# zhenyuw16/Uni3DETR

Hardware: AMD Instinct MI355X
Metric: scenes/sec (fwd+bwd) SUN-RGB-D 20k pts, 300 queries (higher is better)
Workload: dtype bf16

## Files before the change

### include/u3d_hip.h

```cpp
#ifndef U3D_HIP_H_
#define U3D_HIP_H_

#include <stddef.h>
#include <stdint.h>

#ifdef __cplusplus
extern "C" {
#endif

typedef struct ihipStream_t* u3d_stream;

enum {
  U3D_OK = 0,
  U3D_ERR_ARG = -1,
  U3D_ERR_UNSUPPORTED = -2,
  U3D_ERR_LAUNCH = -3,
  U3D_ERR_WORKSPACE = -4
};

enum { U3D_F32 = 0, U3D_BF16 = 1 };

int32_t u3d_version(void);
const char* u3d_strerror(int32_t code);

// ... 59 lines not shown
                             const float voxel_size[3], const float pc_range[6], int32_t* coors, u3d_stream s);
int32_t u3d_scatter_mean(const float* points, const int32_t* rank, int32_t n_total, int32_t nfeat, float* sums,
                         int32_t* counts, int32_t n_voxels, u3d_stream s);

int32_t u3d_spconv_fwd(const void* in, const void* w, const int32_t* nbr, int32_t ld, void* out,
                       const int32_t* n_out_dev, int32_t n_out_cap, int32_t cin, int32_t cout, int32_t kvol,
                       int32_t transpose_w, int32_t dtype, u3d_stream s);

enum { U3D_FWD_EPI_PLAIN, U3D_FWD_EPI_ADD, U3D_FWD_EPI_STATS, U3D_FWD_EPI_AFFINE, U3D_FWD_EPI_COUNT };
enum { U3D_FWD_FAM_NONE, U3D_FWD_FAM_CONV_IN, U3D_FWD_FAM_DIRECT, U3D_FWD_FAM_GLDS, U3D_FWD_FAM_REG, U3D_FWD_FAM_COUNT };
typedef struct u3d_fwd_plan_info {
  int32_t family, kernel, rows, cols, partials, rows_per_partial, takes_addend;
} u3d_fwd_plan_info;
int32_t u3d_igemm_fwd_plan(int32_t n_out_cap, int32_t cin, int32_t cout, int32_t kvol, int32_t has_nbr, int32_t nmajor, int32_t epi,
                           u3d_fwd_plan_info* info);
int32_t u3d_igemm_fwd_bf16(const void* in, const void* w, const int32_t* nbr, int32_t ld, void* out,
                           const int32_t* n_out_dev, int32_t n_out_cap, int32_t cin, int32_t cout, int32_t kvol,
                           int32_t transpose_w, const void* addend, double* stats, u3d_stream s);
int32_t u3d_linear_bf16(const void* x, const void* w, const float* bias, int32_t relu, void* out, const int32_t* m_dev,
                        int32_t m_cap, int32_t k, int32_t n, u3d_stream s);
typedef struct u3d_bn_fold_job {
  const float* w;
  const float* gamma;
  const float* beta;
  const float* mean;
  const float* var;
  uint16_t* w_folded;
  float* shift;
  int64_t sk, sa, sb;
  float eps;
// ... 128 lines not shown
                     const int32_t* n_dev, int32_t n_cap, int32_t c, int32_t dtype, const int32_t* row_map, const void* post_add,
                     u3d_stream s);
int32_t u3d_bn_bwd_stats(const void* dy, const void* y, const void* x, const float* mean, const float* invstd,
                         const float* gamma, const float* beta, int32_t relu, const int32_t* n_dev, int32_t n_cap,
                         int32_t c, int32_t dtype, double* sums, void* workspace, int64_t workspace_bytes,
                         const int32_t* row_map, float* sums_f32, u3d_stream s);
int32_t u3d_bn_bwd_apply(const void* dy, const void* y, const void* x, const float* mean, const float* invstd,
                         const float* gamma, const float* beta, const double* sums, int32_t relu, void* dx, void* dres,
                         const int32_t* n_dev, int32_t n_cap, int32_t c, int32_t dtype, const int32_t* row_map, u3d_stream s);
int32_t u3d_bn_apply_planes(const float* x, const float* mean, const float* invstd, const float* gamma, const float* beta,
                            const float* residual, int32_t relu, float* y, void* planes, const int32_t* n_dev, int32_t n_cap,
                            int32_t c, const int32_t* row_map, const float* post_add, u3d_stream s);
int32_t u3d_bn_bwd_apply_planes(const float* dy, const float* y, const float* x, const float* mean, const float* invstd,
                                const float* gamma, const float* beta, const double* sums, int32_t relu, float* dx, float* dres,
                                void* planes, const int32_t* n_dev, int32_t n_cap, int32_t c, const int32_t* row_map, u3d_stream s);

int32_t u3d_to_dense(const void* feat, const int32_t* coors, const int32_t* n_dev, int32_t n_cap, int32_t c,
                     void* dense, int32_t dz, int32_t dy, int32_t dx, int32_t dtype, u3d_stream s);
int32_t u3d_from_dense(const void* dense, const int32_t* coors, const int32_t* n_dev, int32_t n_cap, int32_t c,
                       void* feat, int32_t dz, int32_t dy, int32_t dx, int32_t dtype, u3d_stream s);

int32_t u3d_gather_rows(const void* in, const int32_t* idx, int32_t n, int32_t row_bytes, void* out, u3d_stream s);
int32_t u3d_scatter_rows(const void* in, const int32_t* idx, int32_t n, int32_t row_bytes, void* out, u3d_stream s);

int32_t u3d_fps(const float* base, const int64_t* set_off, const int32_t* set_n, int32_t nsets, int32_t max_n,
                int32_t m, int32_t* out_idx, float* temp, int64_t temp_stride, int32_t* err, int64_t poll_ticks, int32_t max_wg,
                u3d_stream s);
int32_t u3d_fps2(const float* base, const float* base2, int32_t split, const int64_t* set_off, const int32_t* set_n,
                 int32_t nsets, int32_t max_n, int32_t m, int32_t* out_idx, float* temp, int64_t temp_stride, int32_t* err,
                 int64_t poll_ticks, int32_t max_wg, u3d_stream s);
// ... 337 lines not shown
```

### uni3detr_amd/csrc/igemm_bf16.hip

```cpp
#include "igemm_common.h"
#include "conv_in.h"
#include "igemm_direct.h"

#ifndef IGEMM_SMALL_WM
#define IGEMM_SMALL_WM 4
#endif
#ifndef GLDS256_CFG
#define GLDS256_CFG 2, 4, 8, 4
#endif
#ifndef GLDS_DMA_SPREAD
#define GLDS_DMA_SPREAD 2
#endif
#ifndef GLDS_FRAG_B128
#define GLDS_FRAG_B128 1
#endif
#ifndef IGEMM_STORE_KS
#define IGEMM_STORE_KS 0
#endif

__device__ __forceinline__ bf16x8 direct_frag(const u16* tile, int stride, int r0, int k0, int lane) {
  const int g = lane >> 4, i = lane & 15;
  const u16* p = tile + (r0 + i) * stride + k0 + 4 * g;
  typedef const volatile s16x4 __attribute__((address_space(3))) * lds_vptr;
  s16x4 a = *(lds_vptr)(p);
// ... 835 lines not shown

struct FwdPlan {
  int family = U3D_FWD_FAM_NONE;
  int kernel = 0;
  DirectPlan direct;
  glds_kernel_t fn = nullptr;
  int rows = 0, cols = 0;
  dim3 grid;
  int threads = 0;
  size_t lds = 0;
  int partials = 0, part_rows = 0;
  bool addend = false;
  bool served() const { return family != U3D_FWD_FAM_NONE; }
};

constexpr int GLDS8N_MIN_KTILES = 48;
constexpr int GLDS8N_MIN_WGS = 160;

static FwdPlan fwd_plan(int n_out_cap, int cin, int cout, int kvol, bool has_nbr, bool nmajor, FwdEpi epi) {
  FwdPlan p;
  const bool plain = epi == EPI_PLAIN || epi == EPI_ADD;
  auto tiled = [&](int family, int kernel, int rows, int cols, int threads, size_t lds) {
    p.family = family, p.kernel = kernel, p.rows = rows, p.cols = cols, p.threads = threads, p.lds = lds;
    p.grid = dim3(u3d_cdiv(n_out_cap, rows), u3d_cdiv(cout, cols));
  };
  if (plain && !nmajor && convin_shape(cin, cout, kvol)) {
    tiled(U3D_FWD_FAM_CONV_IN, 0, 256, CONVIN_COUT, 256, 0);
    return p;
  }
  if (plain || epi == EPI_STATS) {
// ... 7 lines not shown
  }
  if (n_out_cap <= 0 || cin <= 0 || cout <= 0) return p;
  const long long tiles256 = u3d_cdiv(n_out_cap, 256);
  if (nmajor && cin % 64 == 0 && cout % 64 == 0) {
    const bool r192 = has_nbr && kvol > 1;
    int g;
    if (epi == EPI_BIAS_RELU)
      g = (cout % 256 == 0 && tiles256 * (cout / 256) >= 128) ? G_256x256
          : (cout % 128 == 0 && tiles256 * (cout / 128) >= 128) ? G_256x128 : G_128x64;
    else if (cout % 256 == 0 && tiles256 * (cout / 256) >= 128)
      g = !has_nbr ? G_256x256 : (r192 && igemm_rows192(n_out_cap, cout / 256)) ? G8_192x256 : G8_256x256;
    else if (has_nbr && cout % 128 == 0 && kvol * (cin / 64) >= GLDS8N_MIN_KTILES && tiles256 * (cout / 128) >= GLDS8N_MIN_WGS)
      g = (r192 && igemm_rows192(n_out_cap, cout / 128)) ? G8_192x128 : G8_256x128;
    else
      g = cout % 128 == 0 ? G_128x128 : G_128x64;
    const GldsKernel& k = GLDS_KERNELS[g];
    p.fn = (epi == EPI_F32 || epi == EPI_F32_ADD) ? k.f32 : k.bf16;
    if (!p.fn) return p;
    tiled(U3D_FWD_FAM_GLDS, g, k.rows, k.cols, k.threads, k.lds);
    p.partials = (int)p.grid.x;
    p.part_rows = k.rows;
    p.addend = k.addend;
    return p;
  }
  if (!plain) return p;
  int r = -1;
  if ((cin == 16 || cin == 32) && (cout == 16 || cout == 32 || cout == 64))
    r = (cout == 16 ? R_N16_K : cout == 32 ? R_N32_K : R_N64_K) + (nmajor ? 1 : 0);
  else if (!nmajor && cin % 64 == 0 && cout % 64 == 0)
    r = cout % 256 == 0 ? (tiles256 * (cout / 256) < 128 ? R_256x128 : R_256x256) : cout % 128 == 0 ? R_256x128 : R_128x64;
// ... 76 lines not shown
```

### uni3detr_amd/csrc/rowops.hip

```cpp
#include "common.h"
#include <type_traits>

typedef unsigned short u16;
__device__ __forceinline__ float ld_elem(const float* p, long long i) { return p[i]; }
__device__ __forceinline__ float ld_elem(const u16* p, long long i) { return __uint_as_float(((unsigned)p[i]) << 16); }
__device__ __forceinline__ void st_elem(float* p, long long i, float v) { p[i] = v; }
__device__ __forceinline__ void st_elem(u16* p, long long i, float v) {
  unsigned u = __float_as_uint(v);
  if ((u & 0x7fffffffu) > 0x7f800000u) { p[i] = (u16)((u >> 16) | 0x40u); return; }
  u += 0x7fffu + ((u >> 16) & 1u);
  p[i] = (u16)(u >> 16);
}

static inline int st_rows_per_block(int n_cap, int c) {
  if (n_cap >= 131072) return c >= 128 ? 256 : 512;
  return n_cap >= 32768 ? 128 : 16;
}

template <typename T> struct VecOf;
template <> struct VecOf<float> { static constexpr int N = 4; };
template <> struct VecOf<u16> { static constexpr int N = 8; };

template <typename T>
__device__ __forceinline__ void load_vec(const T* p, float* out);
// ... 14 lines not shown
template <int V>
__device__ __forceinline__ void load_cols(const float* __restrict__ p, int col0, float* out) {
#pragma unroll
  for (int i = 0; i < V; i += 4) {
    const float4 t = *(const float4*)(p + col0 + i);
    out[i] = t.x; out[i + 1] = t.y; out[i + 2] = t.z; out[i + 3] = t.w;
  }
}
template <int V>
__device__ __forceinline__ void load_cols_d(const double* __restrict__ p, int col0, float scale, float* out) {
#pragma unroll
  for (int i = 0; i < V; i += 2) {
    const double2 t = *(const double2*)(p + col0 + i);
    out[i] = (float)t.x * scale; out[i + 1] = (float)t.y * scale;
  }
}

template <typename T, int MODE>
__global__ __launch_bounds__(256) void k_col_stats_vec(const T* __restrict__ x, const T* __restrict__ dy, const T* __restrict__ y,
                                                       const float* __restrict__ mean, const float* __restrict__ invstd,
                                                       const float* __restrict__ gamma, const float* __restrict__ beta, int relu,
                                                       const int* __restrict__ n_dev, int n_cap, int c, double* __restrict__ partial,
                                                       const int* __restrict__ row_map, int rows_per_block) {
  constexpr int V = VecOf<T>::N;
  extern __shared__ __attribute__((aligned(16))) char smem_raw[];
  double* red = (double*)smem_raw;
  const int n = min(*n_dev, n_cap);
  const int cv = c / V;
  const int cw = cv < 256 ? cv : 256;
  const int rl = 256 / cw;
// ... 18 lines not shown
      for (int r = r0 + trow; r < r1; r += rl) {
        const long long o = (long long)r * c + (long long)vc * V;
        float xv[V];
        load_vec<T>(x + o, xv);
        if (MODE == 0) {
#pragma unroll
          for (int e = 0; e < V; ++e) { s0[e] += xv[e]; s1[e] += xv[e] * xv[e]; }
        } else {
          float gv[V], yv[V];
          const long long oy = row_map ? (long long)row_map[r] * c + (long long)vc * V : o;
          load_vec<T>(dy + oy, gv);
          if (relu && !remask) load_vec<T>(y + oy, yv);
#pragma unroll
          for (int e = 0; e < V; ++e) {
            float g = gv[e];
            if (remask) yv[e] = (xv[e] - mu[e]) * is[e] * ga[e] + be[e];
            if (relu && !(yv[e] > 0.f)) g = 0.f;
            s0[e] += g;
            s1[e] += g * ((xv[e] - mu[e]) * is[e]);
          }
        }
      }
    }
    const int ncol = cw * V;
    if (trow < rl) {
#pragma unroll
      for (int e = 0; e < V; ++e) {
        red[(0 * rl + trow) * ncol + tcol * V + e] = (double)s0[e];
        red[(1 * rl + trow) * ncol + tcol * V + e] = (double)s1[e];
      }
    }
// ... 479 lines not shown
                                                      const int* __restrict__ n_dev, int n_cap, int c, const int* __restrict__ row_map,
                                                      const T* __restrict__ post_add, u16* __restrict__ planes = nullptr) {
  constexpr int V = VecOf<T>::N;
  static_assert(!PLANES || V == 4, "planes are an f32 feature");
  const int n = min(*n_dev, n_cap), cv = c / V, rpb = 256 / cv;
  const int vc = threadIdx.x % cv, rl = threadIdx.x / cv;
  float mu[V], is[V], ga[V], be[V];
  load_cols<V>(mean, vc * V, mu); load_cols<V>(invstd, vc * V, is); load_cols<V>(gamma, vc * V, ga); load_cols<V>(beta, vc * V, be);
  for (int r = blockIdx.x * rpb + rl; r < n; r += gridDim.x * rpb) {
    const long long o = (long long)r * c + (long long)vc * V;
    float xv[V], rv[V], out[V];
    load_vec<T>(x + o, xv);
    if (res) load_vec<T>(res + o, rv);
#pragma unroll
    for (int e = 0; e < V; ++e) {
      float v = (xv[e] - mu[e]) * is[e] * ga[e] + be[e];
      if (res) v += rv[e];
      if (relu) v = v > 0.f ? v : 0.f;
      out[e] = v;
    }
    const long long oy = row_map ? (long long)row_map[r] * c + (long long)vc * V : o;
    if (post_add) {
      float pv[V];
      load_vec<T>(post_add + oy, pv);
#pragma unroll
      for (int e = 0; e < V; ++e) out[e] += pv[e];
    }
    store_vec<T>(y + oy, out);
    if constexpr (PLANES) store_planes4(planes + oy, (long long)n_cap * c, out);
  }
  if constexpr (PLANES) {
// ... 24 lines not shown
    for (int e = 0; e < V; ++e) be[e] = 0.f;
  }
  load_cols_d<V>(sums, vc * V, inv_n, mg);
  load_cols_d<V>(sums + c, vc * V, inv_n, mgx);
#pragma unroll 2
  for (int r = blockIdx.x * rpb + rl; r < n; r += gridDim.x * rpb) {
    const long long o = (long long)r * c + (long long)vc * V;
    float gv[V], xv[V], yv[V], dxv[V];
    const long long oy = row_map ? (long long)row_map[r] * c + (long long)vc * V : o;
    load_vec<T>(dy + oy, gv);
    load_vec<T>(x + o, xv);
    if (relu && !remask) load_vec<T>(y + oy, yv);
#pragma unroll
    for (int e = 0; e < V; ++e) {
      float g = gv[e];
      if (remask) yv[e] = (xv[e] - mu[e]) * is[e] * ga[e] + be[e];
      if (relu && !(yv[e] > 0.f)) g = 0.f;
      const float xh = (xv[e] - mu[e]) * is[e];
      dxv[e] = ga[e] * is[e] * (g - mg[e] - xh * mgx[e]);
      gv[e] = g;
    }
    store_vec<T>(dx + o, dxv);
    if constexpr (PLANES) store_planes4(planes + o, (long long)n_cap * c, dxv);
    if (dres) store_vec<T>(dres + o, gv);
  }
  if constexpr (PLANES) {
    const float z[4] = {0.f, 0.f, 0.f, 0.f};
    for (int r = n + blockIdx.x * rpb + rl; r < n_cap; r += gridDim.x * rpb)
      store_planes4(planes + (long long)r * c + (long long)vc * V, (long long)n_cap * c, z);
  }
}

static inline bool bn_vec_ok(int c, int v) { return c % v == 0 && (c / v) <= 256 && 256 % (c / v) == 0; }
static inline int bn_vec_grid(int n_cap, int c, int v) {
  int rpb = 256 / (c / v);
  long long b = ((long long)n_cap + rpb - 1) / rpb;
  return (int)(b < 1 ? 1 : (b > 2048 ? 2048 : b));
}

static inline int ew_grid(long long total) {
  long long b = (total + 255) / 256;
  return (int)(b < 1 ? 1 : (b > 8192 ? 8192 : b));
}

// ... 53 lines not shown
  U3D_CHECK_LAUNCH();
  return U3D_OK;
}
extern "C" int32_t u3d_bn_bwd_apply_planes(const float* dy, const float* y, const float* x, const float* mean, const float* invstd,
                                           const float* gamma, const float* beta, const double* sums, int32_t relu, float* dx, float* dres,
                                           void* planes, const int32_t* n_dev, int32_t n_cap, int32_t c, const int32_t* row_map, u3d_stream s) {
  U3D_REQUIRE(dy && x && mean && invstd && gamma && sums && dx && planes && n_dev && c > 0 && (!relu || y || beta), U3D_ERR_ARG);
  if (!bn_vec_ok(c, 4) || !(al16(mean) && al16(invstd) && al16(gamma) && al16(beta) && al16(sums)) || (row_map && dres)) return U3D_ERR_UNSUPPORTED;
  if (n_cap <= 0) return U3D_OK;
  hipLaunchKernelGGL((k_bn_bwd_apply_vec<float, true>), dim3(bn_vec_grid(n_cap, c, 4)), dim3(256), 0, s, dy, y, x, mean, invstd, gamma, beta, sums, relu,
                     dx, dres, n_dev, n_cap, c, row_map, (u16*)planes);
  U3D_CHECK_LAUNCH();
  return U3D_OK;
}

template <bool TO_DENSE>
__global__ void k_dense_rows(const uint32_t* __restrict__ src, const int4* __restrict__ coors, const int* __restrict__ n_dev,
                             int n_cap, int row_words, uint32_t* __restrict__ dst, int dz, int dy, int dx) {
  long long total = (long long)min(*n_dev, n_cap) * row_words;
  for (long long t = (long long)blockIdx.x * blockDim.x + threadIdx.x; t < total; t += (long long)gridDim.x * blockDim.x) {
    int r = (int)(t / row_words), w = (int)(t % row_words);
    int4 c = coors[r];
    long long cell = (((long long)c.x * dz + c.y) * dy + c.z) * dx + c.w;
    if (TO_DENSE) dst[cell * row_words + w] = src[t];
    else dst[t] = src[cell * row_words + w];
  }
}

static int run_dense(bool to_dense, const void* a, const int32_t* coors, const int32_t* n_dev, int n_cap, int c, void* b, int dz,
                     int dy, int dx, int dtype, hipStream_t s) {
// ... 320 lines not shown
```

### uni3detr_amd/native.py

```python
import collections
import ctypes as C
import os

import numpy as np
import torch

from . import abi

_HERE = os.path.dirname(os.path.abspath(__file__))
LIB_PATH = os.environ.get("U3D_LIB_PATH") or os.path.join(_HERE, "libu3d_hip.so")

_ABI = abi.load()
_K = _ABI.constants


def _struct(c_name, py_name):
    return abi.structure(_ABI.structs[c_name], py_name)


def _slot_names(prefix):
    names = sorted((v, n[len(prefix):]) for n, v in _K.items() if n.startswith(prefix))
    assert [v for v, _ in names] == list(range(len(names))) and names[-1][1] == "COUNT" and _K[prefix + "COUNT"] == len(names) - 1
    return [n for _, n in names[:-1]]


U3D_ERR_UNSUPPORTED = _K["U3D_ERR_UNSUPPORTED"]
F32, BF16 = _K["U3D_F32"], _K["U3D_BF16"]


class U3DError(RuntimeError):
    pass


BitGridStruct = _struct("u3d_bitgrid", "BitGridStruct")

for _n, _v in _K.items():
    if _n.startswith(("U3D_DL_", "U3D_DLN_")):
        globals()[_n[4:]] = _v
DS_NAMES = _slot_names("U3D_DS_")
DG_NAMES = _slot_names("U3D_DG_")
DecLayerParams = _struct("u3d_declayer_params", "DecLayerParams")
DecLayerDims = _struct("u3d_declayer_dims", "DecLayerDims")
# ... 283 lines not shown
                  "glds_128x64")
FWD_KERNELS = {"conv_in": ("conv_in",), "glds": AFFINE_KERNELS,
               "direct": tuple(f"{s}_{v}" for s in ("32x16", "32x32", "32x64", "64x16", "64x32") for v in ("k", "n", "ns", "nf")),
               "reg": ("n16_k", "n16_n", "n32_k", "n32_n", "n64_k", "n64_n", "256x256", "256x128", "128x64")}
FwdPlanInfo = _struct("u3d_fwd_plan_info", "FwdPlanInfo")
FwdPlan = collections.namedtuple("FwdPlan", "family kernel rows cols partials rows_per_partial takes_addend")


def fwd_plan(n_out, cin, cout, kvol, has_nbr, nmajor, epi="plain"):
    i = FwdPlanInfo()
    rc = lib().u3d_igemm_fwd_plan(n_out, cin, cout, kvol, bool(has_nbr), bool(nmajor), FWD_EPI[epi], C.byref(i))
    if rc:
        return None if rc == U3D_ERR_UNSUPPORTED else _check(rc, "igemm_fwd_plan")
    family = FWD_FAMILIES[i.family]
    return FwdPlan(family, FWD_KERNELS[family][i.kernel], i.rows, i.cols, i.partials, i.rows_per_partial, bool(i.takes_addend))


def fwd_stats_layout(n_out, cin, cout, kvol, has_nbr):
    p = fwd_plan(n_out, cin, cout, kvol, has_nbr, True, "stats")
    return p and (p.partials, p.rows_per_partial)


class SubmHalo:
    TILE = 128

    MAX_ROWS = 140 * 256 * 32

    def __init__(self, nbr_fwd, n_dev, n_cap):
        dev = nbr_fwd.device
        a, b, t = C.c_int64(0), C.c_int64(0), C.c_int32(0)
# ... 665 lines not shown
    if want_planes:
        if x.dtype == torch.float32 and x.is_cuda:
            planes = torch.empty((2 * n, c), dtype=torch.bfloat16, device=x.device)
            rc = lib().u3d_bn_bwd_apply_planes(_ptr(dy), _ptr(y), _ptr(x), _ptr(mean), _ptr(invstd), _ptr(gamma), _ptr(beta), _ptr(sums), int(relu),
                                               _ptr(dx), _ptr(dres), _ptr(planes), _ptr(n_dev), n, c, _ptr(row_map), _stream())
            if rc == 0:
                return dx, dres, planes
            if rc != U3D_ERR_UNSUPPORTED:
                _check(rc, "bn_bwd_apply_planes")
        _check(lib().u3d_bn_bwd_apply(_ptr(dy), _ptr(y), _ptr(x), _ptr(mean), _ptr(invstd), _ptr(gamma), _ptr(beta), _ptr(sums), int(relu),
                                      _ptr(dx), _ptr(dres), _ptr(n_dev), n, c, dtype_code(x), _ptr(row_map), _stream()), "bn_bwd_apply")
        return dx, dres, None
    _check(lib().u3d_bn_bwd_apply(_ptr(dy), _ptr(y), _ptr(x), _ptr(mean), _ptr(invstd), _ptr(gamma), _ptr(beta), _ptr(sums), int(relu),
                                  _ptr(dx), _ptr(dres), _ptr(n_dev), n, c, dtype_code(x), _ptr(row_map), _stream()), "bn_bwd_apply")
    return dx, dres


def to_dense(feat, coors, n_dev, batch, dims):
    n, c = feat.shape
    dz, dy, dx = dims
    vol = torch.zeros((batch, dz, dy, dx, c), dtype=feat.dtype, device=feat.device)
    _check(lib().u3d_to_dense(_ptr(feat), _ptr(coors), _ptr(n_dev), n, c, _ptr(vol), dz, dy, dx, dtype_code(feat), _stream()),
           "to_dense")
    return vol.permute(0, 4, 1, 2, 3)


def from_dense(vol_cl, coors, n_dev, n):
    b, dz, dy, dx, c = vol_cl.shape
    feat = torch.empty((n, c), dtype=vol_cl.dtype, device=vol_cl.device)
    _check(lib().u3d_from_dense(_ptr(vol_cl), _ptr(coors), _ptr(n_dev), n, c, _ptr(feat), dz, dy, dx, dtype_code(vol_cl),
# ... 1080 lines not shown
```

### uni3detr_amd/plugin/dense.py

```python

import numpy as np
import torch
from torch import nn

from .. import native as nv
from .. import sparse as sp
from ..registry import BACKBONES, NECKS


def _conv(cfg, cin, cout, kernel, stride=1, padding=0):
    cfg = dict(cfg)
    t = cfg.pop("type")
    if t != "Conv3d":
        raise NotImplementedError("the HIP dense path implements the Conv3d variant used by every shipped config")
    if cfg.get("bias", True):
        raise NotImplementedError("shipped configs build these convolutions with bias=False")
    return nn.Conv3d(cin, cout, kernel, stride=stride, padding=padding, **cfg)


def _norm(cfg, c):
    cfg = dict(cfg)
    t = cfg.pop("type")
    assert t == "BN3d", "shipped configs use BN3d"
    cfg.pop("requires_grad", None)
# ... 35 lines not shown
            z = torch.arange(D, device=device).view(1, -1, 1, 1)
            y = torch.arange(H * s, device=device).view(1, 1, -1, 1)
            x = torch.arange(W * s, device=device).view(1, 1, 1, -1)
            in_row = ((b * D + z) * H + y // s) * W + x // s
            tap = (y % s) * s + (x % s)
            idx = (in_row * (s * s) + tap).reshape(-1).int().contiguous()
            inv = torch.empty_like(idx)
            inv[idx.long()] = torch.arange(idx.numel(), device=device, dtype=torch.int32)
            v = (idx, inv, (D, H * s, W * s))
            cls._cache[key] = v
        return v


FUSED_LEVEL_SUM = True
FUSED_UPSAMPLE_ORDER = True


class _GatherBijection(torch.autograd.Function):
    @staticmethod
    def forward(ctx, rows, idx, inv):
        ctx.save_for_backward(inv)
        return nv.gather_rows(rows.contiguous(), idx)

    @staticmethod
    def backward(ctx, dout):
        (inv,) = ctx.saved_tensors
        return nv.gather_rows(dout.contiguous(), inv), None, None


def to_rows(x):
    B, C, D, H, W = x.shape
    return x.permute(0, 2, 3, 4, 1).reshape(-1, C), B, (D, H, W)


def to_volume(rows, B, dims):
    return rows.view(B, *dims, rows.shape[1]).permute(0, 4, 1, 2, 3)


def conv_bn_relu(rows, B, dims, conv, bn, post_add=None, fan_token=None):
    ks, st, pd = tuple(conv.kernel_size), tuple(conv.stride), tuple(conv.padding)
    geom, dims_out = Lattice.conv(rows.device, B, dims, ks, st, pd)
    return sp.conv_bn(rows, conv.weight, geom, bn, geom.n_out_dev, None, True, "oidhw", post_add, fan_token=fan_token), dims_out


def deconv_bn_relu(rows, B, dims, deconv, bn, post_add=None):
    s = deconv.stride[1]
    assert tuple(deconv.kernel_size) == (1, s, s) and tuple(deconv.stride) == (1, s, s), "non-overlapping (1,s,s) upsampling only"
    cin, cout = deconv.weight.shape[0], deconv.weight.shape[1]
    n_in = rows.shape[0]
    geom, _ = Lattice.conv(rows.device, B, dims, (1, 1, 1), (1, 1, 1), (0, 0, 0))
    w = deconv.weight.permute(0, 2, 3, 4, 1).reshape(1, 1, 1, cin, s * s * cout)
    y = sp.sparse_conv(rows, w, geom).view(n_in * s * s, cout)
    idx, inv, dims_out = Lattice.upsample_index(rows.device, B, dims, s)
    n_dev = Lattice.conv(rows.device, B, dims_out, (1, 1, 1), (1, 1, 1), (0, 0, 0))[0].n_out_dev
    if FUSED_UPSAMPLE_ORDER:
        return sp.bn_rows(y, bn, n_dev, None, True, row_map=inv, post_add=post_add), dims_out
    y = _GatherBijection.apply(y, idx, inv)
    return sp.bn_rows(y, bn, n_dev, None, True, post_add=post_add), dims_out


FANOUT_FUSION = True


@BACKBONES.register_module()
class SECOND3D(nn.Module):
    def __init__(self, in_channels=128, out_channels=[128, 128, 256], layer_nums=[3, 5, 5], layer_strides=[2, 2, 2],
                 is_cascade=True, norm_cfg=dict(type="BN3d", eps=1e-3, momentum=0.01), conv_cfg=dict(type="Conv3d", bias=False),
                 init_cfg=None, pretrained=None):
        super().__init__()
# ... 82 lines not shown
        self.deblocks = nn.ModuleList(deblocks)
        self.extra_conv = extra_conv
        if extra_conv is not None:
            extra = dict(extra_conv)
            self.layer_num = extra.pop("num_conv")
            kernel = tuple(extra.pop("kernel")) if "kernel" in extra else (3, 3, 3)
            if "sep_kernel" in extra:
                raise NotImplementedError("sep_kernel is not used by any shipped Uni3DETR config")
            padding = tuple((k - 1) // 2 for k in kernel)
            layers = []
            for _ in range(self.layer_num):
                layers += [_conv(extra, out_channels[-1], out_channels[-1], kernel, 1, padding), _norm(norm_cfg, out_channels[-1]),
                           nn.ReLU(inplace=True)]
            self.extra_blocks = nn.Sequential(*layers)

    def forward(self, x):
        assert len(x) == len(self.in_channels)
        out, odims, B = None, None, None
        for i, d in enumerate(self.deblocks):
            rows, B, dims = to_rows(x[i])
            fuse = FUSED_LEVEL_SUM and out is not None and rows.is_cuda and out.dtype == rows.dtype
            if isinstance(d[0], nn.ConvTranspose3d):
                r, dd = deconv_bn_relu(rows, B, dims, d[0], d[1], out if fuse else None)
            else:
                r, dd = conv_bn_relu(rows, B, dims, d[0], d[1], out if fuse else None)
            assert odims is None or odims == dd, "FPN levels must land on one lattice"
            out, odims = (r if (out is None or fuse) else out + r), dd
        if self.extra_conv is not None:
            mods = list(self.extra_blocks)
            for j in range(0, len(mods), 3):
                out, odims = conv_bn_relu(out, B, odims, mods[j], mods[j + 1])
        return to_volume(out, B, odims)
```

### uni3detr_amd/sparse.py

```python
import collections
import contextlib
import os

import torch

from . import native as nv
from .shadow import conv_weights, halo_packs

K3, S1, P1 = (3, 3, 3), (1, 1, 1), (1, 1, 1)


class Level:

    def __init__(self, grid, coords, n, n_dev):
        self.grid, self.coords, self.n, self.n_dev = grid, coords, n, n_dev
        self.dims, self.batch = grid.dims, grid.batch
        self._subm = None
        self._halo = None

    def halo(self):
        if self._halo is None:
            h = nv.SubmHalo(self.subm_tables()[0], self.n_dev, self.n) if self.n <= nv.SubmHalo.MAX_ROWS else None
            self._halo = h if (h is not None and h.ok) else False
        return self._halo or None
# ... 479 lines not shown
    kvol, cout, cin = ent.w_folded.shape
    halo = _halo_of(geom, kvol, cin, cout) if ent.route == "halo" else None
    if residual is not None and halo is None and ent.route != "direct":
        return None
    feats, add = feats.contiguous(), None if residual is None else residual.contiguous()
    nv.CALL_KIND = geom.kind
    if halo is not None:
        return nv.subm_halo_conv_affine(feats, ent.w_packed, halo, ent.shift, relu, add)
    if ent.route == "direct":
        return nv.igemm_direct_affine(feats, ent.w_folded, geom.nbr_fwd, ent.shift, relu, geom.n_out_dev, geom.n_out, add)
    if ent.route == "fp8":
        nv.absmax_rows(feats, geom.n_in_dev, ent.slot)
    return nv.igemm_fwd_affine(feats, ent.w_folded, geom.nbr_fwd if kvol > 1 else None, ent.shift, relu, geom.n_out_dev, geom.n_out)


def conv_bn(feats, weight, geom, bn, n_dev, residual=None, relu=True, layout="dhwio", post_add=None, res_take=None, res_give=None, fan_token=None):
    if _FOLD[0] is not None:
        ent = _FOLD[0].get(id(bn))
        if ent is not None:
            if bn.training or post_add is not None or (residual is not None and not ent.sparse_level):
                what = "an fp8 conv + BatchNorm pair" if ent.route == "fp8" else "a folded conv + BatchNorm pair"
                raise RuntimeError(f"{what} of a sparse level was called in training mode, or with a level sum" if ent.sparse_level else
                                   f"{what} was called in training mode, or with a residual / level sum")
            y = conv_folded(feats, ent, geom, residual, relu)
            if y is not None:
                return y
    if FUSED_CONV_STATS and bn.training and feats.is_cuda and (feats.dtype == torch.bfloat16 or _split_serves(feats, feats.shape[1], bn.num_features) == "wide"):
        y, stats = _SparseConv.apply(feats, weight, geom, layout, True, res_take, fan_token)
        if stats.numel():
            tr = getattr(stats, "_u3d_tile_rows", None)
            if tr is None:
                nb = stats.shape[0]
                tr = next((t for t in (128, 256, 192) if (y.shape[0] + t - 1) // t == nb), 0)
            return _BNRows.apply(y, bn.weight, bn.bias, residual, n_dev, bn, relu, True, stats, tr, None, post_add, res_give)
        return _BNRows.apply(y, bn.weight, bn.bias, residual, n_dev, bn, relu, bn.training, None, 0, None, post_add, res_give)
    return bn_rows(sparse_conv(feats, weight, geom, layout, fan_token), bn, n_dev, residual, relu, None, post_add)


class _BNRows(torch.autograd.Function):

    @staticmethod
    def forward(ctx, x, gamma, beta, residual, n_dev, bn, relu, training, stats=None, tile_rows=0, row_map=None, post_add=None, res_token=None):
        n = x.shape[0]
        if training and stats is not None:
            mean, invstd = nv.bn_finalize_partials(stats, tile_rows, n_dev, n, bn.eps, bn.momentum if bn.momentum is not None else 0.1,
                                                   bn.running_mean, bn.running_var, bn.num_batches_tracked)
        elif training:
            mean, invstd = nv.bn_forward_stats(x, n_dev, bn.eps, bn.momentum if bn.momentum is not None else 0.1,
                                               bn.running_mean, bn.running_var, bn.num_batches_tracked)
        else:
# ... 28 lines not shown
            dx, dres, dpl = nv.bn_bwd_apply(dy, y, x, mean, invstd, gamma, use, ctx.relu, ctx.n_dev, ctx.has_res, beta, ctx.row_map, want_planes=True)
            _give_bwd_planes(dx, dpl)
        else:
            dx, dres = nv.bn_bwd_apply(dy, y, x, mean, invstd, gamma, use, ctx.relu, ctx.n_dev, ctx.has_res, beta, ctx.row_map)
        if ctx.pdtype != torch.float32:
            s32 = s32.to(ctx.pdtype)
        if ctx.res_token is not None and dres is not None:
            ctx.res_token.dres, dres = dres, None
        return dx, s32[1], s32[0], dres, None, None, None, None, None, None, None, (dy if ctx.has_post else None), None


def bn_rows(x, bn, n_dev, residual=None, relu=True, row_map=None, post_add=None):
    return _BNRows.apply(x, bn.weight, bn.bias, residual, n_dev, bn, relu, bn.training, None, 0, row_map, post_add, None)


class _ToDense(torch.autograd.Function):
    @staticmethod
    def forward(ctx, feats, lvl):
        ctx.lvl = lvl
        vol = nv.to_dense(feats, lvl.coords, lvl.n_dev, lvl.batch, lvl.dims)
        ctx.active = _ACTIVE[0] = None
        if ACTIVE_FIRST_CONV and ctx.needs_input_grad[0] and feats.dtype == torch.bfloat16 and feats.is_cuda:
            ctx.set_materialize_grads(False)
            ctx.active = _ACTIVE[0] = ActiveInput(lvl, feats, vol)
        return vol

    @staticmethod
    def backward(ctx, dvol):
        lvl, act = ctx.lvl, ctx.active
        din = None
# ... 42 lines not shown
```

Before: 438.6.

## Fuse FPN level BN-apply, ReLU and sum into one multi-level kernel

Adds kernels that apply BatchNorm and ReLU to up to four FPN levels and sum them in a single pass, plus a matching backward kernel that writes every level's input gradient from one read of the upstream gradient. The neck forward now routes through this merged path in training, so it no longer runs a separate BN-apply and add per level. This cuts separate launches and intermediate activation round-trips through memory, at the cost of holding every level's input for backward. It also adds a short-K kernel override hook for 1x1 convs, which stays inactive unless it is selected.

```diff
diff --git a/include/u3d_hip.h b/include/u3d_hip.h
--- a/include/u3d_hip.h
+++ b/include/u3d_hip.h
@@ -97,6 +97,8 @@
 } u3d_fwd_plan_info;
 int32_t u3d_igemm_fwd_plan(int32_t n_out_cap, int32_t cin, int32_t cout, int32_t kvol, int32_t has_nbr, int32_t nmajor, int32_t epi,
                            u3d_fwd_plan_info* info);
+#define U3D_SHORT_K_PLAN -1
+int32_t u3d_igemm_short_k_select(int32_t kernel);
 int32_t u3d_igemm_fwd_bf16(const void* in, const void* w, const int32_t* nbr, int32_t ld, void* out,
                            const int32_t* n_out_dev, int32_t n_out_cap, int32_t cin, int32_t cout, int32_t kvol,
                            int32_t transpose_w, const void* addend, double* stats, u3d_stream s);
@@ -255,6 +257,14 @@
 int32_t u3d_bn_bwd_apply_planes(const float* dy, const float* y, const float* x, const float* mean, const float* invstd,
                                 const float* gamma, const float* beta, const double* sums, int32_t relu, float* dx, float* dres,
                                 void* planes, const int32_t* n_dev, int32_t n_cap, int32_t c, const int32_t* row_map, u3d_stream s);
+#define U3D_BN_LEVELS_MAX 4
+int32_t u3d_bn_apply_levels(const void* const* x, const float* const* mean, const float* const* invstd, const float* const* gamma,
+                            const float* const* beta, const int32_t* const* src_map, int32_t levels, void* y, const int32_t* n_dev,
+                            int32_t n_cap, int32_t c, int32_t dtype, u3d_stream s);
+int32_t u3d_bn_bwd_apply_levels(const void* dout, const void* const* x, const float* const* mean, const float* const* invstd,
+                                const float* const* gamma, const float* const* beta, const double* const* sums,
+                                const int32_t* const* src_map, void* const* dx, int32_t levels, const int32_t* n_dev, int32_t n_cap,
+                                int32_t c, int32_t dtype, u3d_stream s);
 
 int32_t u3d_to_dense(const void* feat, const int32_t* coors, const int32_t* n_dev, int32_t n_cap, int32_t c,
                      void* dense, int32_t dz, int32_t dy, int32_t dx, int32_t dtype, u3d_stream s);
diff --git a/uni3detr_amd/csrc/igemm_bf16.hip b/uni3detr_amd/csrc/igemm_bf16.hip
--- a/uni3detr_amd/csrc/igemm_bf16.hip
+++ b/uni3detr_amd/csrc/igemm_bf16.hip
@@ -873,6 +873,13 @@
   bool served() const { return family != U3D_FWD_FAM_NONE; }
 };
 
+static int g_short_k = U3D_SHORT_K_PLAN;
+extern "C" int32_t u3d_igemm_short_k_select(int32_t kernel) {
+  U3D_REQUIRE(kernel == U3D_SHORT_K_PLAN || kernel == G_256x256 || kernel == G_256x128 || kernel == G_128x128 || kernel == G_128x64, U3D_ERR_ARG);
+  g_short_k = kernel;
+  return U3D_OK;
+}
+
 constexpr int GLDS8N_MIN_KTILES = 48;
 constexpr int GLDS8N_MIN_WGS = 160;
 
@@ -910,6 +917,9 @@
       g = (r192 && igemm_rows192(n_out_cap, cout / 128)) ? G8_192x128 : G8_256x128;
     else
       g = cout % 128 == 0 ? G_128x128 : G_128x64;
+    if (g_short_k != U3D_SHORT_K_PLAN && !has_nbr && kvol == 1 && cin <= 512 && (plain || epi == EPI_STATS) &&
+        cout % GLDS_KERNELS[g_short_k].cols == 0)
+      g = g_short_k;
     const GldsKernel& k = GLDS_KERNELS[g];
     p.fn = (epi == EPI_F32 || epi == EPI_F32_ADD) ? k.f32 : k.bf16;
     if (!p.fn) return p;
diff --git a/uni3detr_amd/csrc/rowops.hip b/uni3detr_amd/csrc/rowops.hip
--- a/uni3detr_amd/csrc/rowops.hip
+++ b/uni3detr_amd/csrc/rowops.hip
@@ -52,6 +52,12 @@
     const double2 t = *(const double2*)(p + col0 + i);
     out[i] = (float)t.x * scale; out[i + 1] = (float)t.y * scale;
   }
+}
+
+__device__ __forceinline__ float bn_affine(float x, float mu, float is, float ga, float be) { return (x - mu) * is * ga + be; }
+__device__ __forceinline__ float bn_dx(float g, float x, float mu, float is, float ga, float mg, float mgx) {
+  const float xh = (x - mu) * is;
+  return ga * is * (g - mg - xh * mgx);
 }
 
 template <typename T, int MODE>
@@ -100,7 +106,7 @@
 #pragma unroll
           for (int e = 0; e < V; ++e) {
             float g = gv[e];
-            if (remask) yv[e] = (xv[e] - mu[e]) * is[e] * ga[e] + be[e];
+            if (remask) yv[e] = bn_affine(xv[e], mu[e], is[e], ga[e], be[e]);
             if (relu && !(yv[e] > 0.f)) g = 0.f;
             s0[e] += g;
             s1[e] += g * ((xv[e] - mu[e]) * is[e]);
@@ -610,7 +616,7 @@
     if (res) load_vec<T>(res + o, rv);
 #pragma unroll
     for (int e = 0; e < V; ++e) {
-      float v = (xv[e] - mu[e]) * is[e] * ga[e] + be[e];
+      float v = bn_affine(xv[e], mu[e], is[e], ga[e], be[e]);
       if (res) v += rv[e];
       if (relu) v = v > 0.f ? v : 0.f;
       out[e] = v;
@@ -665,10 +671,9 @@
 #pragma unroll
     for (int e = 0; e < V; ++e) {
       float g = gv[e];
-      if (remask) yv[e] = (xv[e] - mu[e]) * is[e] * ga[e] + be[e];
+      if (remask) yv[e] = bn_affine(xv[e], mu[e], is[e], ga[e], be[e]);
       if (relu && !(yv[e] > 0.f)) g = 0.f;
-      const float xh = (xv[e] - mu[e]) * is[e];
-      dxv[e] = ga[e] * is[e] * (g - mg[e] - xh * mgx[e]);
+      dxv[e] = bn_dx(g, xv[e], mu[e], is[e], ga[e], mg[e], mgx[e]);
       gv[e] = g;
     }
     store_vec<T>(dx + o, dxv);
@@ -679,6 +684,119 @@
     const float z[4] = {0.f, 0.f, 0.f, 0.f};
     for (int r = n + blockIdx.x * rpb + rl; r < n_cap; r += gridDim.x * rpb)
       store_planes4(planes + (long long)r * c + (long long)vc * V, (long long)n_cap * c, z);
+  }
+}
+
+template <typename T>
+__device__ __forceinline__ void round_vec(float* v);
+template <>
+__device__ __forceinline__ void round_vec<float>(float*) {}
+template <>
+__device__ __forceinline__ void round_vec<u16>(float* v) {
+  typedef float f32x8_t __attribute__((ext_vector_type(8)));
+  typedef __bf16 bf16x8_t __attribute__((ext_vector_type(8)));
+  const f32x8_t f = {v[0], v[1], v[2], v[3], v[4], v[5], v[6], v[7]};
+  const f32x8_t g = __builtin_convertvector(__builtin_convertvector(f, bf16x8_t), f32x8_t);
+#pragma unroll
+  for (int e = 0; e < 8; ++e) v[e] = g[e];
+}
+
+struct BnLevelsFwd {
+  const void* x[U3D_BN_LEVELS_MAX];
+  const float *mean[U3D_BN_LEVELS_MAX], *invstd[U3D_BN_LEVELS_MAX], *gamma[U3D_BN_LEVELS_MAX], *beta[U3D_BN_LEVELS_MAX];
+  const int* src_map[U3D_BN_LEVELS_MAX];
+};
+struct BnLevelsBwd {
+  const void* x[U3D_BN_LEVELS_MAX];
+  const float *mean[U3D_BN_LEVELS_MAX], *invstd[U3D_BN_LEVELS_MAX], *gamma[U3D_BN_LEVELS_MAX], *beta[U3D_BN_LEVELS_MAX];
+  const double* sums[U3D_BN_LEVELS_MAX];
+  const int* src_map[U3D_BN_LEVELS_MAX];
+  void* dx[U3D_BN_LEVELS_MAX];
+};
+
+template <typename T, int L>
+__global__ __launch_bounds__(256) void k_bn_apply_levels(BnLevelsFwd p, T* __restrict__ y, const int* __restrict__ n_dev, int n_cap, int c) {
+  constexpr int V = VecOf<T>::N;
+  const int n = min(*n_dev, n_cap), cv = c / V, rpb = 256 / cv;
+  const int vc = threadIdx.x % cv, rl = threadIdx.x / cv;
+  const long long col = (long long)vc * V;
+  float mu[L][V], is[L][V], ga[L][V], be[L][V];
+#pragma unroll
+  for (int l = 0; l < L; ++l) {
+    load_cols<V>(p.mean[l], vc * V, mu[l]); load_cols<V>(p.invstd[l], vc * V, is[l]);
+    load_cols<V>(p.gamma[l], vc * V, ga[l]); load_cols<V>(p.beta[l], vc * V, be[l]);
+  }
+  const int step = gridDim.x * rpb;
+  int r = blockIdx.x * rpb + rl;
+  int src[L];
+#pragma unroll
+  for (int l = 0; l < L; ++l) src[l] = (r < n && p.src_map[l]) ? p.src_map[l][r] : r;
+  for (; r < n; r += step) {
+    float xv[L][V], acc[V];
+#pragma unroll
+    for (int l = 0; l < L; ++l) load_vec<T>((const T*)p.x[l] + (long long)src[l] * c + col, xv[l]);
+    const int rn = r + step;
+#pragma unroll
+    for (int l = 0; l < L; ++l) src[l] = (rn < n && p.src_map[l]) ? p.src_map[l][rn] : rn;
+#pragma unroll
+    for (int l = 0; l < L; ++l) {
+#pragma unroll
+      for (int e = 0; e < V; ++e) {
+        float v = bn_affine(xv[l][e], mu[l][e], is[l][e], ga[l][e], be[l][e]);
+        v = v > 0.f ? v : 0.f;
+        acc[e] = l == 0 ? v : v + acc[e];
+      }
+      if (l + 1 < L) round_vec<T>(acc);
+    }
+    store_vec<T>(y + (long long)r * c + col, acc);
+  }
+}
+
+template <typename T, int L>
+__global__ __launch_bounds__(256) void k_bn_bwd_apply_levels(BnLevelsBwd p, const T* __restrict__ dout, const int* __restrict__ n_dev,
+                                                             int n_cap, int c) {
+  constexpr int V = VecOf<T>::N;
+  const int n = min(*n_dev, n_cap), cv = c / V, rpb = 256 / cv;
+  const int vc = threadIdx.x % cv, rl = threadIdx.x / cv;
+  const long long col = (long long)vc * V;
+  const float inv_n = n > 0 ? 1.f / (float)n : 0.f;
+  float mu[L][V], is[L][V], ga[L][V], be[L][V], mg[L][V], mgx[L][V];
+#pragma unroll
+  for (int l = 0; l < L; ++l) {
+    load_cols<V>(p.mean[l], vc * V, mu[l]); load_cols<V>(p.invstd[l], vc * V, is[l]);
+    load_cols<V>(p.gamma[l], vc * V, ga[l]); load_cols<V>(p.beta[l], vc * V, be[l]);
+    load_cols_d<V>(p.sums[l], vc * V, inv_n, mg[l]);
+    load_cols_d<V>(p.sums[l] + c, vc * V, inv_n, mgx[l]);
+  }
+  const int step = gridDim.x * rpb;
+  int r = blockIdx.x * rpb + rl;
+  int src[L];
+#pragma unroll
+  for (int l = 0; l < L; ++l) src[l] = (r < n && p.src_map[l]) ? p.src_map[l][r] : r;
+  for (; r < n; r += step) {
+    float gv[V], xv[L][V];
+    long long o[L];
+    load_vec<T>(dout + (long long)r * c + col, gv);
+#pragma unroll
+    for (int l = 0; l < L; ++l) {
+      o[l] = (long long)src[l] * c + col;
+      load_vec<T>((const T*)p.x[l] + o[l], xv[l]);
+    }
+    const int rn = r + step;
+#pragma unroll
+    for (int l = 0; l < L; ++l) src[l] = (rn < n && p.src_map[l]) ? p.src_map[l][rn] : rn;
+#pragma unroll
+    for (int l = 0; l < L; ++l) {
+      float dxv[V];
+#pragma unroll
+      for (int e = 0; e < V; ++e) {
+        float g = gv[e];
+        const float yv = bn_affine(xv[l][e], mu[l][e], is[l][e], ga[l][e], be[l][e]);
+        if (!(yv > 0.f)) g = 0.f;
+        dxv[e] = bn_dx(g, xv[l][e], mu[l][e], is[l][e], ga[l][e], mg[l][e], mgx[l][e]);
+      }
+      store_vec<T>((T*)p.dx[l] + o[l], dxv);
+    }
   }
 }
 
@@ -762,6 +880,63 @@
   return U3D_OK;
 }
 
+template <typename T, int L>
+static void launch_bn_apply_levels(const BnLevelsFwd& p, void* y, const int32_t* n_dev, int n_cap, int c, u3d_stream s) {
+  hipLaunchKernelGGL((k_bn_apply_levels<T, L>), dim3(bn_vec_grid(n_cap, c, VecOf<T>::N)), dim3(256), 0, s, p, (T*)y, n_dev, n_cap, c);
+}
+template <typename T, int L>
+static void launch_bn_bwd_apply_levels(const BnLevelsBwd& p, const void* dout, const int32_t* n_dev, int n_cap, int c, u3d_stream s) {
+  hipLaunchKernelGGL((k_bn_bwd_apply_levels<T, L>), dim3(bn_vec_grid(n_cap, c, VecOf<T>::N)), dim3(256), 0, s, p, (const T*)dout, n_dev, n_cap, c);
+}
+extern "C" int32_t u3d_bn_apply_levels(const void* const* x, const float* const* mean, const float* const* invstd,
+                                       const float* const* gamma, const float* const* beta, const int32_t* const* src_map, int32_t levels,
+                                       void* y, const int32_t* n_dev, int32_t n_cap, int32_t c, int32_t dtype, u3d_stream s) {
+  U3D_REQUIRE(x && mean && invstd && gamma && beta && src_map && y && n_dev && c > 0 && levels >= 1 && levels <= U3D_BN_LEVELS_MAX, U3D_ERR_ARG);
+  if (!((dtype == U3D_F32 && bn_vec_ok(c, 4)) || (dtype == U3D_BF16 && bn_vec_ok(c, 8)))) return U3D_ERR_UNSUPPORTED;
+  BnLevelsFwd p = {};
+  for (int l = 0; l < levels; ++l) {
+    U3D_REQUIRE(x[l] && mean[l] && invstd[l] && gamma[l] && beta[l], U3D_ERR_ARG);
+    U3D_REQUIRE(al16(x[l]) && al16(mean[l]) && al16(invstd[l]) && al16(gamma[l]) && al16(beta[l]), U3D_ERR_ARG);
+    p.x[l] = x[l]; p.mean[l] = mean[l]; p.invstd[l] = invstd[l]; p.gamma[l] = gamma[l]; p.beta[l] = beta[l]; p.src_map[l] = src_map[l];
+  }
+  U3D_REQUIRE(al16(y), U3D_ERR_ARG);
+  if (n_cap <= 0) return U3D_OK;
+  typedef void (*Fn)(const BnLevelsFwd&, void*, const int32_t*, int, int, u3d_stream);
+  static const Fn f32[U3D_BN_LEVELS_MAX] = {launch_bn_apply_levels<float, 1>, launch_bn_apply_levels<float, 2>, launch_bn_apply_levels<float, 3>,
+                                            launch_bn_apply_levels<float, 4>};
+  static const Fn b16[U3D_BN_LEVELS_MAX] = {launch_bn_apply_levels<u16, 1>, launch_bn_apply_levels<u16, 2>, launch_bn_apply_levels<u16, 3>,
+                                            launch_bn_apply_levels<u16, 4>};
+  (dtype == U3D_F32 ? f32 : b16)[levels - 1](p, y, n_dev, n_cap, c, s);
+  U3D_CHECK_LAUNCH();
+  return U3D_OK;
+}
+
+extern "C" int32_t u3d_bn_bwd_apply_levels(const void* dout, const void* const* x, const float* const* mean, const float* const* invstd,
+                                           const float* const* gamma, const float* const* beta, const double* const* sums,
+                                           const int32_t* const* src_map, void* const* dx, int32_t levels, const int32_t* n_dev,
+                                           int32_t n_cap, int32_t c, int32_t dtype, u3d_stream s) {
+  U3D_REQUIRE(dout && x && mean && invstd && gamma && beta && sums && src_map && dx && n_dev && c > 0 && levels >= 1 &&
+              levels <= U3D_BN_LEVELS_MAX, U3D_ERR_ARG);
+  if (!((dtype == U3D_F32 && bn_vec_ok(c, 4)) || (dtype == U3D_BF16 && bn_vec_ok(c, 8)))) return U3D_ERR_UNSUPPORTED;
+  BnLevelsBwd p = {};
+  for (int l = 0; l < levels; ++l) {
+    U3D_REQUIRE(x[l] && mean[l] && invstd[l] && gamma[l] && beta[l] && sums[l] && dx[l], U3D_ERR_ARG);
+    U3D_REQUIRE(al16(x[l]) && al16(dx[l]) && al16(mean[l]) && al16(invstd[l]) && al16(gamma[l]) && al16(beta[l]) && al16(sums[l]), U3D_ERR_ARG);
+    p.x[l] = x[l]; p.mean[l] = mean[l]; p.invstd[l] = invstd[l]; p.gamma[l] = gamma[l]; p.beta[l] = beta[l]; p.sums[l] = sums[l];
+    p.src_map[l] = src_map[l]; p.dx[l] = dx[l];
+  }
+  U3D_REQUIRE(al16(dout), U3D_ERR_ARG);
+  if (n_cap <= 0) return U3D_OK;
+  typedef void (*Fn)(const BnLevelsBwd&, const void*, const int32_t*, int, int, u3d_stream);
+  static const Fn f32[U3D_BN_LEVELS_MAX] = {launch_bn_bwd_apply_levels<float, 1>, launch_bn_bwd_apply_levels<float, 2>,
+                                            launch_bn_bwd_apply_levels<float, 3>, launch_bn_bwd_apply_levels<float, 4>};
+  static const Fn b16[U3D_BN_LEVELS_MAX] = {launch_bn_bwd_apply_levels<u16, 1>, launch_bn_bwd_apply_levels<u16, 2>,
+                                            launch_bn_bwd_apply_levels<u16, 3>, launch_bn_bwd_apply_levels<u16, 4>};
+  (dtype == U3D_F32 ? f32 : b16)[levels - 1](p, dout, n_dev, n_cap, c, s);
+  U3D_CHECK_LAUNCH();
+  return U3D_OK;
+}
+
 template <bool TO_DENSE>
 __global__ void k_dense_rows(const uint32_t* __restrict__ src, const int4* __restrict__ coors, const int* __restrict__ n_dev,
                              int n_cap, int row_words, uint32_t* __restrict__ dst, int dz, int dy, int dx) {
diff --git a/uni3detr_amd/native.py b/uni3detr_amd/native.py
--- a/uni3detr_amd/native.py
+++ b/uni3detr_amd/native.py
@@ -26,6 +26,7 @@
 
 U3D_ERR_UNSUPPORTED = _K["U3D_ERR_UNSUPPORTED"]
 F32, BF16 = _K["U3D_F32"], _K["U3D_BF16"]
+U3D_BN_LEVELS_MAX = _K["U3D_BN_LEVELS_MAX"]
 
 
 class U3DError(RuntimeError):
@@ -339,6 +340,10 @@
         return None if rc == U3D_ERR_UNSUPPORTED else _check(rc, "igemm_fwd_plan")
     family = FWD_FAMILIES[i.family]
     return FwdPlan(family, FWD_KERNELS[family][i.kernel], i.rows, i.cols, i.partials, i.rows_per_partial, bool(i.takes_addend))
+
+
+def short_k_select(kernel=None):
+    _check(lib().u3d_igemm_short_k_select(_K["U3D_SHORT_K_PLAN"] if kernel is None else AFFINE_KERNELS.index(kernel)), "igemm_short_k_select")
 
 
 def fwd_stats_layout(n_out, cin, cout, kvol, has_nbr):
@@ -1034,6 +1039,41 @@
     _check(lib().u3d_bn_bwd_apply(_ptr(dy), _ptr(y), _ptr(x), _ptr(mean), _ptr(invstd), _ptr(gamma), _ptr(beta), _ptr(sums), int(relu),
                                   _ptr(dx), _ptr(dres), _ptr(n_dev), n, c, dtype_code(x), _ptr(row_map), _stream()), "bn_bwd_apply")
     return dx, dres
+
+
+def _opt_ptr_array(tensors):
+    arr = (C.c_void_p * len(tensors))()
+    for i, t in enumerate(tensors):
+        assert t is None or (t.is_cuda and t.is_contiguous()), "device-contiguous tensor required"
+        arr[i] = None if t is None else t.data_ptr()
+    return arr
+
+
+def _levels_args(xs, per_level):
+    n, c = xs[0].shape
+    if not 1 <= len(xs) <= U3D_BN_LEVELS_MAX or any(len(a) != len(xs) for a in per_level):
+        raise ValueError(f"a level merge takes 1..{U3D_BN_LEVELS_MAX} levels with one entry per level in every list")
+    if any(x.shape != xs[0].shape or x.dtype != xs[0].dtype for x in xs):
+        raise ValueError("the levels of a merge are row matrices of one shape and dtype")
+    return n, c
+
+
+def bn_apply_levels(xs, means, invstds, gammas, betas, src_maps, n_dev, out=None):
+    n, c = _levels_args(xs, (means, invstds, gammas, betas, src_maps))
+    y = torch.empty_like(xs[0]) if out is None else out
+    _check(lib().u3d_bn_apply_levels(_opt_ptr_array(xs), _opt_ptr_array(means), _opt_ptr_array(invstds), _opt_ptr_array(gammas),
+                                     _opt_ptr_array(betas), _opt_ptr_array(src_maps), len(xs), _ptr(y), _ptr(n_dev), n, c,
+                                     dtype_code(xs[0]), _stream()), "bn_apply_levels")
+    return y
+
+
+def bn_bwd_apply_levels(dout, xs, means, invstds, gammas, betas, sums, src_maps, n_dev, out=None):
+    n, c = _levels_args(xs, (means, invstds, gammas, betas, sums, src_maps))
+    dxs = [torch.empty_like(x) for x in xs] if out is None else out
+    _check(lib().u3d_bn_bwd_apply_levels(_ptr(dout), _opt_ptr_array(xs), _opt_ptr_array(means), _opt_ptr_array(invstds),
+                                         _opt_ptr_array(gammas), _opt_ptr_array(betas), _opt_ptr_array(sums), _opt_ptr_array(src_maps),
+                                         _opt_ptr_array(dxs), len(xs), _ptr(n_dev), n, c, dtype_code(xs[0]), _stream()), "bn_bwd_apply_levels")
+    return dxs
 
 
 def to_dense(feat, coors, n_dev, batch, dims):
diff --git a/uni3detr_amd/plugin/dense.py b/uni3detr_amd/plugin/dense.py
--- a/uni3detr_amd/plugin/dense.py
+++ b/uni3detr_amd/plugin/dense.py
@@ -73,6 +73,7 @@
 
 FUSED_LEVEL_SUM = True
 FUSED_UPSAMPLE_ORDER = True
+FUSED_LEVEL_APPLY = True
 
 
 class _GatherBijection(torch.autograd.Function):
@@ -96,13 +97,16 @@
     return rows.view(B, *dims, rows.shape[1]).permute(0, 4, 1, 2, 3)
 
 
-def conv_bn_relu(rows, B, dims, conv, bn, post_add=None, fan_token=None):
+def conv_bn_relu(rows, B, dims, conv, bn, post_add=None, fan_token=None, raw=False):
     ks, st, pd = tuple(conv.kernel_size), tuple(conv.stride), tuple(conv.padding)
     geom, dims_out = Lattice.conv(rows.device, B, dims, ks, st, pd)
+    if raw:
+        y, stats, tr = sp.conv_bn(rows, conv.weight, geom, bn, geom.n_out_dev, None, True, "oidhw", fan_token=fan_token, raw=True)
+        return (y, bn, None, stats, tr), dims_out
     return sp.conv_bn(rows, conv.weight, geom, bn, geom.n_out_dev, None, True, "oidhw", post_add, fan_token=fan_token), dims_out
 
 
-def deconv_bn_relu(rows, B, dims, deconv, bn, post_add=None):
+def deconv_bn_relu(rows, B, dims, deconv, bn, post_add=None, raw=False):
     s = deconv.stride[1]
     assert tuple(deconv.kernel_size) == (1, s, s) and tuple(deconv.stride) == (1, s, s), "non-overlapping (1,s,s) upsampling only"
     cin, cout = deconv.weight.shape[0], deconv.weight.shape[1]
@@ -112,6 +116,8 @@
     y = sp.sparse_conv(rows, w, geom).view(n_in * s * s, cout)
     idx, inv, dims_out = Lattice.upsample_index(rows.device, B, dims, s)
     n_dev = Lattice.conv(rows.device, B, dims_out, (1, 1, 1), (1, 1, 1), (0, 0, 0))[0].n_out_dev
+    if raw:
+        return (y, bn, (idx, inv), None, 0), dims_out
     if FUSED_UPSAMPLE_ORDER:
         return sp.bn_rows(y, bn, n_dev, None, True, row_map=inv, post_add=post_add), dims_out
     y = _GatherBijection.apply(y, idx, inv)
@@ -224,10 +230,32 @@
                            nn.ReLU(inplace=True)]
             self.extra_blocks = nn.Sequential(*layers)
 
+    def _merged_apply(self, x):
+        t = x[0]
+        c = self.out_channels[0]
+        return (FUSED_LEVEL_APPLY and FUSED_LEVEL_SUM and FUSED_UPSAMPLE_ORDER and 2 <= len(x) <= nv.U3D_BN_LEVELS_MAX
+                and all(v.is_cuda and v.dtype == t.dtype for v in x) and t.dtype in (torch.bfloat16, torch.float32)
+                and all(oc == c for oc in self.out_channels) and sp._FOLD[0] is None and all(d[1].training for d in self.deblocks)
+                and not (sp.BN_PLANES and sp._SPLIT[0] and t.dtype == torch.float32 and c % 16 == 0))
+
+    def _levels_merged(self, x):
+        levels, odims, B = [], None, None
+        for i, d in enumerate(self.deblocks):
+            rows, B, dims = to_rows(x[i])
+            lv, dd = (deconv_bn_relu if isinstance(d[0], nn.ConvTranspose3d) else conv_bn_relu)(rows, B, dims, d[0], d[1], raw=True)
+            assert odims is None or odims == dd, "FPN levels must land on one lattice"
+            levels.append(lv)
+            odims = dd
+        n_dev = Lattice.conv(levels[0][0].device, B, odims, (1, 1, 1), (1, 1, 1), (0, 0, 0))[0].n_out_dev
+        return sp.bn_level_sum(levels, n_dev), B, odims
+
     def forward(self, x):
         assert len(x) == len(self.in_channels)
         out, odims, B = None, None, None
-        for i, d in enumerate(self.deblocks):
+        merged = self._merged_apply(x)
+        if merged:
+            out, B, odims = self._levels_merged(x)
+        for i, d in enumerate(() if merged else self.deblocks):
             rows, B, dims = to_rows(x[i])
             fuse = FUSED_LEVEL_SUM and out is not None and rows.is_cuda and out.dtype == rows.dtype
             if isinstance(d[0], nn.ConvTranspose3d):
diff --git a/uni3detr_amd/sparse.py b/uni3detr_amd/sparse.py
--- a/uni3detr_amd/sparse.py
+++ b/uni3detr_amd/sparse.py
@@ -517,10 +517,13 @@
     return nv.igemm_fwd_affine(feats, ent.w_folded, geom.nbr_fwd if kvol > 1 else None, ent.shift, relu, geom.n_out_dev, geom.n_out)
 
 
-def conv_bn(feats, weight, geom, bn, n_dev, residual=None, relu=True, layout="dhwio", post_add=None, res_take=None, res_give=None, fan_token=None):
+def conv_bn(feats, weight, geom, bn, n_dev, residual=None, relu=True, layout="dhwio", post_add=None, res_take=None, res_give=None, fan_token=None,
+            raw=False):
     if _FOLD[0] is not None:
         ent = _FOLD[0].get(id(bn))
         if ent is not None:
+            if raw:
+                raise RuntimeError("a folded conv + BatchNorm pair has no raw convolution output")
             if bn.training or post_add is not None or (residual is not None and not ent.sparse_level):
                 what = "an fp8 conv + BatchNorm pair" if ent.route == "fp8" else "a folded conv + BatchNorm pair"
                 raise RuntimeError(f"{what} of a sparse level was called in training mode, or with a level sum" if ent.sparse_level else
@@ -535,8 +538,14 @@
             if tr is None:
                 nb = stats.shape[0]
                 tr = next((t for t in (128, 256, 192) if (y.shape[0] + t - 1) // t == nb), 0)
+            if raw:
+                return y, stats, tr
             return _BNRows.apply(y, bn.weight, bn.bias, residual, n_dev, bn, relu, True, stats, tr, None, post_add, res_give)
+        if raw:
+            return y, None, 0
         return _BNRows.apply(y, bn.weight, bn.bias, residual, n_dev, bn, relu, bn.training, None, 0, None, post_add, res_give)
+    if raw:
+        return sparse_conv(feats, weight, geom, layout, fan_token), None, 0
     return bn_rows(sparse_conv(feats, weight, geom, layout, fan_token), bn, n_dev, residual, relu, None, post_add)
 
 
@@ -595,6 +604,58 @@
     return _BNRows.apply(x, bn.weight, bn.bias, residual, n_dev, bn, relu, bn.training, None, 0, row_map, post_add, None)
 
 
+class _BNLevelSum(torch.autograd.Function):
+
+    @staticmethod
+    def forward(ctx, n_dev, bns, maps, stats, tile_rows, *flat):
+        xs, gammas, betas = flat[0::3], flat[1::3], flat[2::3]
+        n = xs[0].shape[0]
+        means, invstds = [], []
+        for x, bn, st, tr in zip(xs, bns, stats, tile_rows):
+            if not bn.training:
+                raise RuntimeError("the level merge runs on batch statistics: an eval-mode BatchNorm keeps its own apply pass (bn_rows)")
+            mom = bn.momentum if bn.momentum is not None else 0.1
+            if st is not None:
+                mean, invstd = nv.bn_finalize_partials(st, tr, n_dev, n, bn.eps, mom, bn.running_mean, bn.running_var, bn.num_batches_tracked)
+            else:
+                mean, invstd = nv.bn_forward_stats(x, n_dev, bn.eps, mom, bn.running_mean, bn.running_var, bn.num_batches_tracked)
+            means.append(mean); invstds.append(invstd)
+        g32, b32 = [g.float() for g in gammas], [b.float() for b in betas]
+        y = nv.bn_apply_levels(list(xs), means, invstds, g32, b32, [None if m is None else m[0] for m in maps], n_dev)
+        ctx.save_for_backward(*xs, *means, *invstds, *g32, *b32, *[t for m in maps if m is not None for t in m])
+        ctx.n_dev, ctx.levels, ctx.has_map = n_dev, len(xs), [m is not None for m in maps]
+        ctx.pdtype = [g.dtype for g in gammas]
+        return y
+
+    @staticmethod
+    def backward(ctx, dy):
+        L, sv = ctx.levels, ctx.saved_tensors
+        xs, means, invstds, gammas, betas = (list(sv[i * L:(i + 1) * L]) for i in range(5))
+        given = list(sv[5 * L:])
+        maps, rmaps = [None] * L, [None] * L
+        for l in range(L):
+            if ctx.has_map[l]:
+                maps[l], rmaps[l] = given.pop(0), given.pop(0)
+        dy = dy.contiguous()
+        use, s32s = [None] * L, [None] * L
+        for l in reversed(range(L)):
+            use[l], s32 = nv.bn_bwd_stats(dy, None, xs[l], means[l], invstds[l], True, ctx.n_dev, gammas[l], betas[l], rmaps[l], want_f32=True)
+            s32s[l] = s32 if ctx.pdtype[l] == torch.float32 else s32.to(ctx.pdtype[l])
+        dxs = nv.bn_bwd_apply_levels(dy, xs, means, invstds, gammas, betas, use, maps, ctx.n_dev)
+        out = [None] * 5
+        for l in range(L):
+            out += [dxs[l], s32s[l][1], s32s[l][0]]
+        return tuple(out)
+
+
+def bn_level_sum(levels, n_dev):
+    flat = []
+    for x, bn, _, _, _ in levels:
+        flat += [x, bn.weight, bn.bias]
+    return _BNLevelSum.apply(n_dev, [lv[1] for lv in levels], [lv[2] for lv in levels], [lv[3] for lv in levels],
+                             [lv[4] for lv in levels], *flat)
+
+
 class _ToDense(torch.autograd.Function):
     @staticmethod
     def forward(ctx, feats, lvl):
```

New measurement: 439.7 (median of 6 runs). No clear change (+0.2%).
